# craston/object_detection_cib

Hardware: AMD Instinct MI355X
Metric: images/sec YOLOv5s 640px train (higher is better)
Workload: dtype bf16; 1 GPU; yv5s coco-zipf-like synthetic, 640px, bf16 storage/fp32 accumulate, batch 64/GPU, fwd+assign+loss+bwd+SGD, targets 4-30 boxes/img; global_batch=64, parallelism=dp1, launch=hipGraph replay, collectives=none, launcher=none, attempt=0

## Files before the change

object_detection_cib_amd/csrc/bn_act.hip:

```cpp
#include "kodhip_common.h"
#include <stdlib.h>

namespace {

__device__ __forceinline__ double wave_sum_partials(const float* p, int T, int lane) {
  double a0 = 0.0, a1 = 0.0, a2 = 0.0, a3 = 0.0;
  const int T4 = ((reinterpret_cast<uintptr_t>(p) & 15) == 0) ? (T & ~3) : 0;
#pragma unroll 4
  for (int t = lane * 4; t < T4; t += 256) {
    f32x4 v = *reinterpret_cast<const f32x4*>(p + t);
    a0 += (double)v[0]; a1 += (double)v[1]; a2 += (double)v[2]; a3 += (double)v[3];
  }
  for (int t = T4 + lane; t < T; t += 64) a0 += (double)p[t];
  return wave_sum_d((a0 + a1) + (a2 + a3));
}

__device__ __forceinline__ void wave_sum_partials2(const float* p, const float* q, int T, int lane, double& sp, double& sq) {
  const bool al = ((reinterpret_cast<uintptr_t>(p) | reinterpret_cast<uintptr_t>(q)) & 15) == 0;
  if (!al || T > 4 * 256) {
    sp = wave_sum_partials(p, T, lane);
    sq = wave_sum_partials(q, T, lane);
    return;
  }
  const int T4 = T & ~3;
// ... 59 lines not shown

__device__ __forceinline__ float bn_affine(double var, float eps, float g, float b, double mean, float* scale, float* shift) {
  float rstd = (float)(1.0 / sqrt(var + (double)eps));
  float sc = g * rstd;
  *scale = sc;
  *shift = b - (float)mean * sc;
  return rstd;
}

__device__ __forceinline__ void bn_finalize_channel(double s0, double s1, double count, float g, float b, float rm0, float rv0,
                                                    float momentum, float eps, int update_running, int c, float* scale,
                                                    float* shift, float* mean_out, float* rstd_out, float* running_mean,
                                                    float* running_var) {
  double mean = s0 / count;
  double var = s1 / count - mean * mean;
  if (var < 0.0) var = 0.0;
  float rstd = bn_affine(var, eps, g, b, mean, &scale[c], &shift[c]);
  mean_out[c] = (float)mean;
  rstd_out[c] = rstd;
  if (update_running) {
    double unbiased = count > 1.0 ? var * count / (count - 1.0) : var;
    running_mean[c] = (1.f - momentum) * rm0 + momentum * (float)mean;
    running_var[c] = (1.f - momentum) * rv0 + momentum * (float)unbiased;
  }
}

__device__ __forceinline__ double bn_central_moment(double rs, double mu, double s0, double s1) { return rs * (s1 - mu * s0); }

struct BnCoef { float k1, k2, k3; };
__device__ __forceinline__ void bn_coef_store(float* coef, int C, int c, BnCoef k) {
  coef[c] = k.k1;
  coef[C + c] = k.k2;
  coef[2 * C + c] = k.k3;
}

__device__ __forceinline__ BnCoef bn_coef_train(double g, double rs, double mu, double s0, double s1, double count) {
  double S0 = s0 / count, S1 = s1 / count;
  return {(float)(g * rs), (float)(-g * rs * rs * S1), (float)(-g * rs * S0 + g * rs * rs * mu * S1)};
}

__device__ __forceinline__ BnCoef bn_coef_eval(float g, float rstd) { return {(float)((double)g * (double)rstd), 0.f, 0.f}; }

__global__ void bn_finalize_kernel(const double* sums, double count, const float* gamma, const float* beta,
                                   float* running_mean, float* running_var, float momentum, float eps,
                                   float* scale, float* shift, float* mean_out, float* rstd_out, int C,
                                   int update_running) {
  int c = blockIdx.x * blockDim.x + threadIdx.x;
  if (c >= C) return;
  bn_finalize_channel(sums[c], sums[C + c], count, gamma[c], beta[c], update_running ? running_mean[c] : 0.f,
                      update_running ? running_var[c] : 0.f, momentum, eps, update_running, c, scale, shift, mean_out,
                      rstd_out, running_mean, running_var);
}

template <bool PEER>
__global__ void bn_finalize_fused_kernel(const float* part, int T, double count, const float* gamma,
                                         const float* beta, float* running_mean, float* running_var,
                                         float momentum, float eps, float* scale, float* shift, float* mean_out,
                                         float* rstd_out, int C, int update_running, KodPeerView pv, unsigned int slot) {
  int c = blockIdx.x * (blockDim.x >> 6) + (threadIdx.x >> 6);
  if (c >= C) return;
  int lane = threadIdx.x & 63;
  const float* p0 = part + (size_t)c * T;
  const float* p1 = part + (size_t)(C + c) * T;
  const float g = gamma[c], b = beta[c];
  const float rm0 = update_running ? running_mean[c] : 0.f, rv0 = update_running ? running_var[c] : 0.f;
  double s0, s1;
  wave_sum_partials2(p0, p1, T, lane, s0, s1);
  if constexpr (PEER) peer_allreduce2(pv, slot, c, C + c, lane, s0, s1);
  if (lane != 0) return;
  bn_finalize_channel(s0, s1, count, g, b, rm0, rv0, momentum, eps, update_running, c, scale, shift, mean_out, rstd_out,
                      running_mean, running_var);
}

struct CoefJob { const float* part; int T; double count; const float* gamma; const float* mean; const float* rstd;
                 float* dgamma; float* dbeta; float* coef; int C; int raw_moment; int eval; };

template <bool PEER>
__device__ __forceinline__ void bn_bwd_coeffs_channel(const float* part, int T, double count, const float* gamma,
                                                      const float* mean, const float* rstd, float* dgamma, float* dbeta,
                                                      float* coef, int C, int raw_moment, int eval, int c, int lane,
                                                      const KodPeerView& pv, unsigned int slot) {
  const float* p0 = part + (size_t)c * T;
  const float* p1 = part + (size_t)(C + c) * T;
  const float g_ = gamma[c], rs_ = rstd[c], mu_ = mean[c];
  double s0, s1;
  wave_sum_partials2(p0, p1, T, lane, s0, s1);
  if (raw_moment) s1 = bn_central_moment((double)rs_, (double)mu_, s0, s1);
  if (lane == 0) {
    dbeta[c] = (float)s0;
    dgamma[c] = (float)s1;
  }
  if constexpr (PEER) peer_allreduce2(pv, slot, c, C + c, lane, s0, s1);
  if (lane != 0) return;
  BnCoef k = bn_coef_train(g_, rs_, mu_, s0, s1, count);
  if (!PEER && eval) k = bn_coef_eval(g_, rs_);
  bn_coef_store(coef, C, c, k);
}

template <bool PEER>
__global__ void bn_bwd_coeffs_fused_kernel(CoefJob j0, CoefJob j1, KodPeerView pv, unsigned int slot) {
  const CoefJob& j = blockIdx.y == 0 ? j0 : j1;
  int c = blockIdx.x * (blockDim.x >> 6) + (threadIdx.x >> 6);
  if (c >= j.C) return;
  bn_bwd_coeffs_channel<PEER>(j.part, j.T, j.count, j.gamma, j.mean, j.rstd, j.dgamma, j.dbeta, j.coef, j.C, j.raw_moment,
                              j.eval, c, threadIdx.x & 63, pv, slot);
}

struct BnEvalDesc {
  const float* gamma; const float* beta; const float* running_mean; const float* running_var;
  float* aff; float* coef; long long C; long long reserved;
};

__global__ __launch_bounds__(256) void bn_eval_constants_kernel(const BnEvalDesc* desc, float eps) {
  const BnEvalDesc d = desc[blockIdx.x];
  const int C = (int)d.C;
  for (int c = threadIdx.x; c < C; c += blockDim.x) {
    const float g = d.gamma[c], b = d.beta[c], rm = d.running_mean[c];
    const float rstd = bn_affine((double)d.running_var[c], eps, g, b, (double)rm, &d.aff[c], &d.aff[C + c]);
    d.aff[2 * C + c] = rm;
    d.aff[3 * C + c] = rstd;
    if (d.coef != nullptr) bn_coef_store(d.coef, C, c, bn_coef_eval(g, rstd));
  }
}

constexpr int U = 4;

template <int ACT, int U, bool LDSK, int MAXT>
__global__ __launch_bounds__(MAXT) void bn_silu_apply_kernel(const bf16_t* y, int ldy, const float* scale, const float* shift,
                                     const bf16_t* res, int ldr, int rcoff,
                                     bf16_t* out, int ldo, int ocoff, long M, int C, int rows_per_block_iter, float slope) {
  extern __shared__ float kconst[];
  const int CC = C >> 3;
  const int cc = threadIdx.x % CC;
  const int rl = threadIdx.x / CC;
  float sc[8], sh[8];
  if (LDSK) {
    for (int c = threadIdx.x; c < C; c += blockDim.x) { kconst[c] = scale[c]; kconst[C + c] = shift[c]; }
    __syncthreads();
#pragma unroll
    for (int e = 0; e < 8; ++e) { sc[e] = kconst[cc * 8 + e]; sh[e] = kconst[C + cc * 8 + e]; }
  }
  if (rl >= rows_per_block_iter) return;
  if (!LDSK) {
#pragma unroll
    for (int e = 0; e < 8; ++e) { sc[e] = scale[cc * 8 + e]; sh[e] = shift[cc * 8 + e]; }
  }
  const long step = (long)gridDim.x * rows_per_block_iter * U;
  for (long m0 = (long)blockIdx.x * rows_per_block_iter * U + rl; m0 < M; m0 += step) {
    bf16x8 v[U], r[U];
#pragma unroll
    for (int u = 0; u < U; ++u) {
      const long m = m0 + (long)u * rows_per_block_iter;
      if (m < M) {
        v[u] = kod_load_once<bf16x8>(y + m * ldy + cc * 8);
        if (res) r[u] = *reinterpret_cast<const bf16x8*>(res + m * ldr + rcoff + cc * 8);
      }
    }
#pragma unroll
// ... 190 lines not shown
  int rpb = max_threads / CC;
  int q = 1;
  while ((q * C * 2) % 128) q *= 2;
  if (rpb >= q) rpb -= rpb % q;
  if (rpb < 1) rpb = 1;
  Geo g;
  g.rpb = rpb;
  g.threads = ((rpb * CC + 63) / 64) * 64;
  long blocks = (M + (long)rpb * U - 1) / ((long)rpb * U);
  g.grid = (int)(blocks < max_blocks ? blocks : max_blocks);
  if (g.grid < 1) g.grid = 1;
  return g;
}

#define KOD_APPLY_DISPATCH(L)                                                                              \
  do {                                                                                                     \
    const bool big = g.threads > 256;                                                                      \
    if (a.u == 4) { if (a.lds) L(4, true, 256); else L(4, false, 256); }                                   \
    else if (a.u == 2) { if (big) { if (a.lds) L(2, true, 1024); else L(2, false, 1024); }                 \
                         else { if (a.lds) L(2, true, 256); else L(2, false, 256); } }                     \
    else { if (big) { if (a.lds) L(1, true, 1024); else L(1, false, 1024); }                               \
           else { if (a.lds) L(1, true, 256); else L(1, false, 256); } }                                   \
  } while (0)

}

extern "C" {

int kodhip_bn_reduce_partials(const float* partials, double* sums, int C, int T, hipStream_t stream) {
  KOD_CHECK_ARG(partials && sums && C > 0 && T > 0, "bn_reduce_partials: bad args");
  hipLaunchKernelGGL(bn_reduce_partials_kernel, dim3(cdiv(2 * C, 4)), dim3(256), 0, stream, partials, sums, C, T);
  KOD_LAUNCH_CHECK("bn_reduce_partials");
  return KOD_OK;
}

int kodhip_bn_finalize(const double* sums, double count, const float* gamma, const float* beta,
                       float* running_mean, float* running_var, float momentum, float eps,
                       float* scale, float* shift, float* mean, float* rstd, int C, int update_running,
                       hipStream_t stream) {
  KOD_CHECK_ARG(sums && gamma && beta && scale && shift && mean && rstd && C > 0 && count > 0, "bn_finalize: bad args");
  KOD_CHECK_ARG(!update_running || (running_mean && running_var), "bn_finalize: running stats missing");
  hipLaunchKernelGGL(bn_finalize_kernel, dim3(cdiv(C, 64)), dim3(64), 0, stream, sums, count, gamma, beta,
                     running_mean, running_var, momentum, eps, scale, shift, mean, rstd, C, update_running);
  KOD_LAUNCH_CHECK("bn_finalize");
  return KOD_OK;
}

static int bn_finalize_partials(const char* fn, const float* partials, int T, double count, const float* gamma,
                                const float* beta, float* running_mean, float* running_var, float momentum, float eps,
                                float* scale, float* shift, float* mean, float* rstd, int C, int update_running,
                                const void* view, unsigned int slot, hipStream_t stream) {
  KOD_CHECK_ARG(partials && gamma && beta && scale && shift && mean && rstd && C > 0 && T > 0 && count > 0, "%s: bad args", fn);
  KOD_CHECK_ARG(!update_running || (running_mean && running_var), "%s: running stats missing", fn);
  const dim3 grid(cdiv(C, 4)), blk(256);
  if (view) {
    const KodPeerView pv = *(const KodPeerView*)view;
    KOD_CHECK_ARG(pv.world >= 1 && pv.world <= KOD_PEER_MAX && pv.world * 4 <= 64, "%s: bad peer view", fn);
    hipLaunchKernelGGL(bn_finalize_fused_kernel<true>, grid, blk, 0, stream, partials, T, count, gamma, beta, running_mean,
                       running_var, momentum, eps, scale, shift, mean, rstd, C, update_running, pv, slot);
  } else {
    hipLaunchKernelGGL(bn_finalize_fused_kernel<false>, grid, blk, 0, stream, partials, T, count, gamma, beta, running_mean,
                       running_var, momentum, eps, scale, shift, mean, rstd, C, update_running, KodPeerView{}, 0u);
  }
  KOD_LAUNCH_CHECK(fn);
  return KOD_OK;
}

static int bn_bwd_coeffs_partials(const char* fn, const CoefJob* jobs, int n_jobs, const void* view, unsigned int slot,
                                  hipStream_t stream) {
  int Cmax = 0;
  for (int i = 0; i < n_jobs; ++i) {
    const CoefJob& j = jobs[i];
    KOD_CHECK_ARG(j.part && j.gamma && j.mean && j.rstd && j.dgamma && j.dbeta && j.coef && j.C > 0 && j.T > 0 &&
                  (j.eval || j.count > 0), "%s: bad args", fn);
    if (j.C > Cmax) Cmax = j.C;
  }
  const dim3 grid(cdiv(Cmax, 4), n_jobs), blk(256);
  const CoefJob& j1 = jobs[n_jobs - 1];
  if (view) {
    const KodPeerView pv = *(const KodPeerView*)view;
    KOD_CHECK_ARG(pv.world >= 1 && pv.world <= KOD_PEER_MAX, "%s: bad peer view", fn);
    hipLaunchKernelGGL(bn_bwd_coeffs_fused_kernel<true>, grid, blk, 0, stream, jobs[0], j1, pv, slot);
  } else {
    hipLaunchKernelGGL(bn_bwd_coeffs_fused_kernel<false>, grid, blk, 0, stream, jobs[0], j1, KodPeerView{}, 0u);
  }
  KOD_LAUNCH_CHECK(fn);
  return KOD_OK;
}

int kodhip_bn_finalize_partials(const float* partials, int T, double count, const float* gamma, const float* beta,
                                float* running_mean, float* running_var, float momentum, float eps,
                                float* scale, float* shift, float* mean, float* rstd, int C, int update_running,
                                hipStream_t stream) {
  return bn_finalize_partials("bn_finalize_partials", partials, T, count, gamma, beta, running_mean, running_var, momentum, eps,
                              scale, shift, mean, rstd, C, update_running, nullptr, 0u, stream);
}

int kodhip_bn_finalize_partials_peer(const float* partials, int T, double count, const float* gamma, const float* beta,
                                     float* running_mean, float* running_var, float momentum, float eps,
                                     float* scale, float* shift, float* mean, float* rstd, int C, int update_running,
                                     const void* view, unsigned int slot, hipStream_t stream) {
  KOD_CHECK_ARG(view, "bn_finalize_partials_peer: bad args");
  return bn_finalize_partials("bn_finalize_partials_peer", partials, T, count, gamma, beta, running_mean, running_var, momentum,
                              eps, scale, shift, mean, rstd, C, update_running, view, slot, stream);
}

int kodhip_bn_bwd_coeffs_partials_peer(const float* partials, int T, double count, const float* gamma, const float* mean,
                                       const float* rstd, float* dgamma, float* dbeta, float* coef, int C,
                                       int raw_moment, const void* view, unsigned int slot, hipStream_t stream) {
  KOD_CHECK_ARG(view, "bn_bwd_coeffs_partials_peer: bad args");
  const CoefJob j = {partials, T, count, gamma, mean, rstd, dgamma, dbeta, coef, C, raw_moment, 0};
  return bn_bwd_coeffs_partials("bn_bwd_coeffs_partials_peer", &j, 1, view, slot, stream);
}

int kodhip_bn_bwd_coeffs_partials(const float* partials, int T, double count, const float* gamma, const float* mean,
                                  const float* rstd, float* dgamma, float* dbeta, float* coef, int C,
                                  int raw_moment, hipStream_t stream) {
  const CoefJob j = {partials, T, count, gamma, mean, rstd, dgamma, dbeta, coef, C, raw_moment, 0};
  return bn_bwd_coeffs_partials("bn_bwd_coeffs_partials", &j, 1, nullptr, 0u, stream);
}

int kodhip_bn_bwd_coeffs_partials2(const float* partials0, int T0, double count0, const float* gamma0, const float* mean0,
                                   const float* rstd0, float* dgamma0, float* dbeta0, float* coef0, int C0, int raw_moment0,
                                   const float* partials1, int T1, double count1, const float* gamma1, const float* mean1,
                                   const float* rstd1, float* dgamma1, float* dbeta1, float* coef1, int C1, int raw_moment1,
                                   hipStream_t stream) {
  const CoefJob j[2] = {{partials0, T0, count0, gamma0, mean0, rstd0, dgamma0, dbeta0, coef0, C0, raw_moment0, 0},
                        {partials1, T1, count1, gamma1, mean1, rstd1, dgamma1, dbeta1, coef1, C1, raw_moment1, 0}};
  return bn_bwd_coeffs_partials("bn_bwd_coeffs_partials2", j, 2, nullptr, 0u, stream);
}
// ... 144 lines not shown
```

object_detection_cib_amd/csrc/loss.hip:

```cpp
#include "kodhip_common.h"
#include "kodhip_iou.h"
#include <limits.h>

namespace {

struct AssignLevel {
  int* idx;
  int* label;
  float* gt;
  float* anc;
  int* count;
  float aw[3], ah[3];
  float fmap_w, fmap_h;
  int fw, fh;
  double inv_stride;
};
struct AssignArgs {
  AssignLevel lv[3];
  const double* boxes;
  const long* labels;
  const int* samples;
  int n, cap;
  float threshold;
};
// ... 319 lines not shown
    }
  }
  float s = block_sum_256(acc, sm);
  if (threadIdx.x == 0) a.partials[((size_t)(lvl * 3 + 1)) * a.nblk + blockIdx.x] = s;
}

__global__ void loss_scatter_kernel(LossArgs a) {
  const LossLevel& L = a.lv[blockIdx.y];
  const int m = min(*L.count, a.cap);
  int r = blockIdx.x * blockDim.x + threadIdx.x;
  if (r >= m) return;
  const int cell = cell_of(L, a.A, a.cap, r);
  if (L.last[cell] != r) return;
  const int W = 4 + a.nc;
  float* g = L.grad + (size_t)cell * a.P;
  int rows[8];
  int cnt = 0, done = -1;
  for (;;) {
    int nxt = INT_MAX;
    for (int q = L.first[cell]; q >= 0; q = L.prev[q])
      if (q > done && q < nxt) nxt = q;
    if (nxt == INT_MAX) break;
#pragma unroll
    for (int i = 0; i < 8; ++i)
      if (i == cnt) rows[i] = nxt;
    ++cnt;
    done = nxt;
  }
  if (cnt <= 8) {
    for (int k = 0; k < W; ++k) {
      float s = 0.f;
#pragma unroll
      for (int i = 0; i < 8; ++i)
        if (i < cnt) s += L.G[(size_t)rows[i] * W + k];
      g[k < 4 ? k : k + 1] = s;
    }
  } else {
    for (int k = 0; k < W; ++k) {
      float s = 0.f;
      int d2 = -1;
      for (;;) {
        int nxt = INT_MAX;
        for (int q = L.first[cell]; q >= 0; q = L.prev[q])
          if (q > d2 && q < nxt) nxt = q;
        if (nxt == INT_MAX) break;
        s += L.G[(size_t)nxt * W + k];
        d2 = nxt;
      }
      g[k < 4 ? k : k + 1] = s;
    }
  }
}

__global__ void loss_finalize_kernel(LossArgs a, int nblk_rows, int nblk_cells) {
  const int lane = threadIdx.x;
  double box = 0, obj = 0, cls = 0;
  for (int l = 0; l < 3; ++l) {
    const LossLevel& L = a.lv[l];
    double sb = 0, so = 0, sc = 0;
    for (int i = lane; i < nblk_rows; i += 64) {
      sb += (double)a.partials[(size_t)(l * 3 + 0) * a.nblk + i];
      sc += (double)a.partials[(size_t)(l * 3 + 2) * a.nblk + i];
    }
    for (int i = lane; i < nblk_cells; i += 64) so += (double)a.partials[(size_t)(l * 3 + 1) * a.nblk + i];
    sb = wave_sum_d(sb); sc = wave_sum_d(sc); so = wave_sum_d(so);
    int m = min(*L.count, a.cap);
    double ncells = (double)a.B * a.A * L.fh * L.fw;
    float lb = (float)(sb / (double)m);
    float lc = (float)(sc / ((double)m * a.nc));
    float lo = L.balance * (float)(so / ncells);
    if (lane == 0) { a.out[3 + l * 3 + 0] = lb; a.out[3 + l * 3 + 1] = lo; a.out[3 + l * 3 + 2] = lc; }
    box += lb; obj += lo; cls += lc;
  }
  if (lane == 0) {
    const float o0 = a.lam_box * (float)box, o1 = a.lam_obj * (float)obj, o2 = a.lam_cls * (float)cls;
    a.out[0] = o0;
    a.out[1] = o1;
    a.out[2] = o2;
    if (a.upstream) a.out[12] = a.upstream[0] * ((o0 + o2) + o1);
  }
}

}

extern "C" {

struct KodAssignLevel {
  int* idx; int* label; float* gt; float* anc; int* count;
  float anchor_w[3], anchor_h[3];
  int stride;
};

int kodhip_assign_targets(const double* boxes, const long* labels, const int* samples, int n, int cap,
                          int img_w, int img_h, float threshold, const KodAssignLevel* levels ,
                          hipStream_t stream) {
  KOD_CHECK_ARG(levels && cap > 0 && n >= 0, "assign_targets: bad args");
  KOD_CHECK_ARG(n == 0 || (boxes && labels && samples), "assign_targets: null inputs");
  AssignArgs a = {};
  for (int l = 0; l < 3; ++l) {
    const KodAssignLevel& s = levels[l];
    KOD_CHECK_ARG(s.idx && s.label && s.gt && s.anc && s.count && s.stride > 0, "assign_targets: bad level %d", l);
    AssignLevel& d = a.lv[l];
    d.idx = s.idx; d.label = s.label; d.gt = s.gt; d.anc = s.anc; d.count = s.count;
    for (int k = 0; k < 3; ++k) { d.aw[k] = s.anchor_w[k]; d.ah[k] = s.anchor_h[k]; }
    d.fmap_w = (float)((double)img_w / s.stride); d.fmap_h = (float)((double)img_h / s.stride);
    d.fw = img_w / s.stride; d.fh = img_h / s.stride;
    d.inv_stride = 1.0 / (double)s.stride;
  }
  a.boxes = boxes; a.labels = labels; a.samples = samples; a.n = n; a.cap = cap; a.threshold = threshold;
  hipLaunchKernelGGL(assign_kernel, dim3(3), dim3(1024), 0, stream, a);
  KOD_LAUNCH_CHECK("assign_targets");
  return KOD_OK;
}

struct KodLossLevel {
  const float* logits; float* grad;
  const int* idx; const int* label; const float* gt; const float* anc; const int* count;
  int* cellmaps;
  int* rowprev;
  float* rowgrad;
  float* tobj;
  int fh, fw;
  float balance;
};

int kodhip_yolo_loss_iou(const KodLossLevel* levels, int B, int A, int nc, int cap, float lam_box, float lam_obj, float lam_cls,
                         const float* pos_weight, const float* upstream, float* partials, int nslots, float* out,
// ... 3 lines not shown
                     float lam_box, float lam_obj, float lam_cls, const float* pos_weight,
                     const float* upstream, float* partials, int nslots, float* out, int compute_grad,
                     hipStream_t stream) {
  return kodhip_yolo_loss_iou(levels, B, A, nc, cap, lam_box, lam_obj, lam_cls, pos_weight, upstream, partials, nslots, out,
                              compute_grad, 3, 1e-7f, stream);
}

int kodhip_yolo_loss_iou(const KodLossLevel* levels , int B, int A, int nc, int cap,
                         float lam_box, float lam_obj, float lam_cls, const float* pos_weight,
                         const float* upstream, float* partials, int nslots, float* out, int compute_grad,
                         int iou_kind, float iou_eps, hipStream_t stream) {
  KOD_CHECK_ARG(levels && partials && out && B > 0 && A > 0 && nc > 0 && cap > 0, "yolo_loss: bad args");
  KOD_CHECK_ARG(iou_kind >= 0 && iou_kind <= 3 && iou_eps >= 0.f, "yolo_loss: bad IoU kind %d / eps", iou_kind);
  LossArgs a = {};
  a.iou_kind = iou_kind; a.iou_eps = iou_eps; a.iou_generic = !(iou_kind == 3 && iou_eps == 1e-7f);
  long max_cells = 0;
  for (int l = 0; l < 3; ++l) {
    const KodLossLevel& s = levels[l];
    KOD_CHECK_ARG(s.logits && s.idx && s.label && s.gt && s.anc && s.count && s.cellmaps && s.rowprev && s.rowgrad && s.tobj,
                  "yolo_loss: null pointer in level %d", l);
    KOD_CHECK_ARG(!compute_grad || s.grad, "yolo_loss: grad buffer missing");
    long ncells = (long)B * A * s.fh * s.fw;
    KOD_CHECK_ARG(ncells * (5 + nc) < (1l << 31), "yolo_loss: level too large");
    LossLevel& d = a.lv[l];
    d.logits = s.logits; d.grad = s.grad; d.idx = s.idx; d.label = s.label; d.gt = s.gt; d.anc = s.anc;
    d.count = s.count; d.last = s.cellmaps; d.first = s.cellmaps + ncells; d.cnt = s.cellmaps + 2 * ncells;
    d.G = s.rowgrad; d.tobj = s.tobj; d.prev = s.rowprev; d.fh = s.fh; d.fw = s.fw; d.balance = s.balance;
    if (ncells > max_cells) max_cells = ncells;
  }
  int nblk_rows = cdiv(cap, 256);
  int nblk_cells = 1024;
  KOD_CHECK_ARG(nslots >= nblk_rows && nslots >= nblk_cells, "yolo_loss: partials too small (%d)", nslots);
  a.B = B; a.A = A; a.nc = nc; a.P = 5 + nc; a.cap = cap;
  a.lam_box = lam_box; a.lam_obj = lam_obj; a.lam_cls = lam_cls;
  a.pos_weight = pos_weight; a.upstream = upstream; a.partials = partials; a.nblk = nslots; a.out = out;
  a.compute_grad = compute_grad;
  KOD_CHECK_ARG(5 + nc <= 128, "yolo_loss: at most 123 classes");
  a.magic_p = magic_u32((uint32_t)(5 + nc));
  for (int l = 0; l < 3; ++l) {
    long ncells = (long)B * A * a.lv[l].fh * a.lv[l].fw;
    hipError_t e1 = hipMemsetAsync(a.lv[l].last, 0xFF, 2 * ncells * sizeof(int), stream);
    if (e1 != hipSuccess) { kodhip_set_error("yolo_loss: memset failed"); return 1; }
  }
  hipLaunchKernelGGL(loss_mark_kernel, dim3(nblk_rows, 3), dim3(256), 0, stream, a);
  KOD_LAUNCH_CHECK("loss_mark");
  hipLaunchKernelGGL(loss_rows_kernel, dim3(nblk_rows, 3), dim3(256), 0, stream, a);
  KOD_LAUNCH_CHECK("loss_rows");
  hipLaunchKernelGGL(loss_cells_kernel, dim3(nblk_cells, 3), dim3(256), 0, stream, a);
  KOD_LAUNCH_CHECK("loss_cells");
  if (compute_grad) {
    hipLaunchKernelGGL(loss_scatter_kernel, dim3(nblk_rows, 3), dim3(256), 0, stream, a);
    KOD_LAUNCH_CHECK("loss_scatter");
  }
  hipLaunchKernelGGL(loss_finalize_kernel, dim3(1), dim3(64), 0, stream, a, nblk_rows, nblk_cells);
  KOD_LAUNCH_CHECK("loss_finalize");
  return KOD_OK;
}

}
```

object_detection_cib_amd/csrc/misc_ops.hip:

```cpp
#include "kodhip_common.h"

namespace {

__global__ void nchw_to_nhwc4_kernel(const float* x, bf16_t* y, int B, int C, long HW) {
  long i = (long)blockIdx.x * blockDim.x + threadIdx.x;
  if (i >= (long)B * HW) return;
  long b = i / HW, p = i - b * HW;
  bf16x4 v;
#pragma unroll
  for (int c = 0; c < 4; ++c) v[c] = (bf16_t)(c < C ? x[(b * C + c) * HW + p] : 0.f);
  *reinterpret_cast<bf16x4*>(y + i * 4) = v;
}

__global__ void nchw_to_nhwc4_x4_kernel(const float* x, bf16_t* y, int B, int C, long HW) {
  const long q = (long)blockIdx.x * blockDim.x + threadIdx.x;
  const long HWq = HW >> 2;
  if (q >= (long)B * HWq) return;
  const long b = q / HWq, pq = q - b * HWq;
  f32x4 pl[4];
#pragma unroll
  for (int c = 0; c < 4; ++c)
    pl[c] = c < C ? kod_load_once<f32x4>(x + (b * C + c) * HW + pq * 4) : f32x4{0.f, 0.f, 0.f, 0.f};
  bf16x8 o0, o1;
  const float* f0 = reinterpret_cast<const float*>(&pl[0]);
// ... 323 lines not shown

__global__ __launch_bounds__(256) void maxpool_k_bwd_kernel(const bf16_t* dy, int ldy, int ycoff, const unsigned char* idx,
                                                            bf16_t* dx, int ldx, int xcoff, int B, int H, int W, int C, int K,
                                                            const float* dx32) {
  const int C8 = C >> 3;
  const long i = (long)blockIdx.x * blockDim.x + threadIdx.x;
  if (i >= (long)B * H * W * C8) return;
  const int c8 = (int)(i % C8);
  const long p = i / C8;
  const int ix = (int)(p % W), iy = (int)((p / W) % H), b = (int)(p / ((long)W * H));
  const int r = K >> 1;
  float acc[8];
  bf16_t* d = dx + p * ldx + xcoff + c8 * 8;
  if (dx32) {
#pragma unroll
    for (int e = 0; e < 8; ++e) acc[e] = dx32[p * ldx + xcoff + c8 * 8 + e];
  } else {
    const bf16x8 old = *reinterpret_cast<const bf16x8*>(d);
#pragma unroll
    for (int e = 0; e < 8; ++e) acc[e] = (float)old[e];
  }
  for (int oy = max(iy - r, 0); oy <= min(iy + r, H - 1); ++oy)
    for (int ox = max(ix - r, 0); ox <= min(ix + r, W - 1); ++ox) {
      const long q = (long)(b * H + oy) * W + ox;
      const unsigned long long ib = *reinterpret_cast<const unsigned long long*>(idx + q * C + c8 * 8);
      const bf16x8 g = *reinterpret_cast<const bf16x8*>(dy + q * ldy + ycoff + c8 * 8);
      const unsigned me = (unsigned)((iy - oy + r) * 16 + (ix - ox + r));
#pragma unroll
      for (int e = 0; e < 8; ++e)
        if (((ib >> (8 * e)) & 0xffu) == me) acc[e] += (float)g[e];
    }
  bf16x8 o;
#pragma unroll
  for (int e = 0; e < 8; ++e) o[e] = (bf16_t)acc[e];
  *reinterpret_cast<bf16x8*>(d) = o;
}

__global__ void upsample2x_fwd_kernel(const bf16_t* x, int ldx, int xcoff, bf16_t* y, int ldy, int ycoff,
                                      int B, int H, int W, int C) {
  const int CC = C >> 3;
  long i = (long)blockIdx.x * blockDim.x + threadIdx.x;
  long total = (long)B * 4 * H * W * CC;
  if (i >= total) return;
  int cc = (int)(i % CC);
  long p = i / CC;
  int ox = (int)(p % (2 * W));
  long q = p / (2 * W);
  int oy = (int)(q % (2 * H));
  int b = (int)(q / (2 * H));
  bf16x8 v = *reinterpret_cast<const bf16x8*>(x + ((long)(b * H + (oy >> 1)) * W + (ox >> 1)) * ldx + xcoff + cc * 8);
  *reinterpret_cast<bf16x8*>(y + p * ldy + ycoff + cc * 8) = v;
}

__global__ void upsample2x_bwd_kernel(const bf16_t* dy, int ldy, int ycoff, bf16_t* dx, int ldx, int xcoff,
                                      int accumulate, int B, int H, int W, int C, const float* dx32) {
  const int CC = C >> 3;
  long i = (long)blockIdx.x * blockDim.x + threadIdx.x;
  long total = (long)B * H * W * CC;
  if (i >= total) return;
  int cc = (int)(i % CC);
  long p = i / CC;
  int ix = (int)(p % W);
  long q = p / W;
  int iy = (int)(q % H);
  int b = (int)(q / H);
  float acc[8];
  bf16_t* d = dx + p * ldx + xcoff + cc * 8;
  if (accumulate && dx32) {
    const float* o32 = dx32 + p * ldx + xcoff + cc * 8;
#pragma unroll
    for (int e = 0; e < 8; ++e) acc[e] = o32[e];
  } else if (accumulate) {
    bf16x8 old = *reinterpret_cast<const bf16x8*>(d);
#pragma unroll
    for (int e = 0; e < 8; ++e) acc[e] = (float)old[e];
  } else {
#pragma unroll
    for (int e = 0; e < 8; ++e) acc[e] = 0.f;
  }
#pragma unroll
  for (int s = 0; s < 4; ++s) {
    long op = (long)(b * 2 * H + 2 * iy + (s >> 1)) * (2 * W) + 2 * ix + (s & 1);
    bf16x8 g = *reinterpret_cast<const bf16x8*>(dy + op * ldy + ycoff + cc * 8);
#pragma unroll
    for (int e = 0; e < 8; ++e) acc[e] += (float)g[e];
  }
  bf16x8 o;
#pragma unroll
  for (int e = 0; e < 8; ++e) o[e] = (bf16_t)acc[e];
  *reinterpret_cast<bf16x8*>(d) = o;
}

__global__ __launch_bounds__(256) void head_bwd_prep_kernel(const float* g, bf16_t* dy, float* bpart, int B, int HW,
                                                            int A, int nc, int Npad, uint32_t magic_p, int PREP_ROWS) {
  extern __shared__ float sm[];
  const int P = 5 + nc;
  const int N = A * P;
  const int ldt = Npad + 1;
  const long M = (long)B * HW;
  const int ntiles = (int)((M + PREP_ROWS - 1) / PREP_ROWS);
  float bsum = 0.f;
  for (int i = threadIdx.x; i < PREP_ROWS * ldt; i += blockDim.x) sm[i] = 0.f;
  __syncthreads();
  for (int t = blockIdx.x; t < ntiles; t += gridDim.x) {
    const long m0 = (long)t * PREP_ROWS;
    const int b0 = (int)(m0 / HW), pix0 = (int)(m0 - (long)b0 * HW);
    constexpr int UNR = 4;
    const int per_an = PREP_ROWS * P;
    for (int an = 0; an < A; ++an)
      for (int base = 0; base < per_an; base += UNR * blockDim.x) {
        float v[UNR];
        int dst[UNR];
#pragma unroll
        for (int u = 0; u < UNR; ++u) {
          const int idx = base + u * blockDim.x + threadIdx.x;
          v[u] = 0.f; dst[u] = -1;
          if (idx < per_an) {
            const int r = (int)__umulhi((uint32_t)idx, magic_p);
            const int slot = idx - r * P;
            if (m0 + r < M) {
              int b = b0, pix = pix0 + r;
              while (pix >= HW) { pix -= HW; ++b; }
              v[u] = g[(((long)b * A + an) * HW + pix) * P + slot];
            }
            dst[u] = r * ldt + (slot < 4 ? 4 * an + slot : (slot == 4 ? 4 * A + an : 5 * A + an * nc + slot - 5));
          }
        }
#pragma unroll
        for (int u = 0; u < UNR; ++u)
          if (dst[u] >= 0) sm[dst[u]] = v[u];
      }
    __syncthreads();
    const int cpr = Npad / 8;
    for (int c = threadIdx.x; c < PREP_ROWS * cpr; c += blockDim.x) {
      const int r = c / cpr, n0 = (c - r * cpr) * 8;
      if (m0 + r < M) {
        bf16x8 o;
#pragma unroll
        for (int e = 0; e < 8; ++e) o[e] = (bf16_t)sm[r * ldt + n0 + e];
        *reinterpret_cast<bf16x8*>(dy + (m0 + r) * Npad + n0) = o;
      }
    }
    if (threadIdx.x < Npad) {
      float s = 0.f;
      for (int r = 0; r < PREP_ROWS; ++r) s += sm[r * ldt + threadIdx.x];
      bsum += s;
    }
    __syncthreads();
  }
  if (threadIdx.x < Npad) bpart[(size_t)blockIdx.x * Npad + threadIdx.x] = bsum;
  (void)N;
}

__global__ void head_bias_reduce_kernel(const float* bpart, int nblk, int Npad, float* db_box, float* db_obj,
                                        float* db_cls, int A, int nc) {
  int n = blockIdx.x * (blockDim.x >> 6) + (threadIdx.x >> 6);
  int lane = threadIdx.x & 63;
  int N = A * (5 + nc);
  if (n >= N) return;
  double s = 0.0;
  for (int b = lane; b < nblk; b += 64) s += (double)bpart[(size_t)b * Npad + n];
  s = wave_sum_d(s);
  if (lane != 0) return;
  if (n < 4 * A) db_box[n] = (float)s;
  else if (n < 5 * A) db_obj[n - 4 * A] = (float)s;
  else db_cls[n - 5 * A] = (float)s;
}

#define KOD_CLIP_FLOATS 16
#define KOD_NORM_BLOCKS 1024
enum { KOD_CLIP_NONE = -1, KOD_CLIP_NORM = 0, KOD_CLIP_VALUE = 1 };

template <bool NT>
__global__ __launch_bounds__(256) void grad_norm_partial_kernel(const float* __restrict__ g, const unsigned char* __restrict__ gid,
                                                                const unsigned char* __restrict__ count, long n,
                                                                const float* __restrict__ hyper, double* __restrict__ part) {
  const float gscale = hyper[9];
  double s0 = 0.0, s1 = 0.0, s2 = 0.0;
  const long stride = (long)gridDim.x * 256 * 4;
  for (long i0 = ((long)blockIdx.x * 256 + threadIdx.x) * 4; i0 < n; i0 += 4 * stride) {
    f32x4 gv[4];
    unsigned int kv[4];
    unsigned char grp[4];
#pragma unroll
    for (int u = 0; u < 4; ++u) {
      const long i = i0 + u * stride;
      const bool in = i < n;
      const long ic = in ? i : 0;
      grp[u] = gid[ic >> 6];
      kv[u] = count ? *reinterpret_cast<const unsigned int*>(count + ic) : 0x01010101u;
      gv[u] = NT ? kod_load_once<f32x4>(g + ic) : *reinterpret_cast<const f32x4*>(g + ic);
      if (!in || grp[u] > 2) kv[u] = 0;
    }
#pragma unroll
    for (int u = 0; u < 4; ++u) {
      double t = 0.0;
#pragma unroll
      for (int e = 0; e < 4; ++e) {
        const double d = (double)(gv[u][e] * gscale);
        t += ((kv[u] >> (8 * e)) & 0xffu) ? d * d : 0.0;
      }
      s0 += grp[u] == 0 ? t : 0.0;
      s1 += grp[u] == 1 ? t : 0.0;
      s2 += grp[u] == 2 ? t : 0.0;
    }
  }
  __shared__ double sm[3][4];
  s0 = wave_sum_d(s0); s1 = wave_sum_d(s1); s2 = wave_sum_d(s2);
  const int wave = threadIdx.x >> 6;
  if ((threadIdx.x & 63) == 0) { sm[0][wave] = s0; sm[1][wave] = s1; sm[2][wave] = s2; }
  __syncthreads();
  if (threadIdx.x < 3)
    part[(size_t)blockIdx.x * 3 + threadIdx.x] = (sm[threadIdx.x][0] + sm[threadIdx.x][1]) + (sm[threadIdx.x][2] + sm[threadIdx.x][3]);
}
// ... 120 lines not shown
  return KOD_OK;
}

int kodhip_maxpool5_bwd(const void* dy, int ldy, int ycoff, const void* idx, void* dx, int ldx, int xcoff,
                        int B, int H, int W, int C, const float* dx_f32, hipStream_t stream) {
  KOD_CHECK_ARG(dy && dx && idx && C % 8 == 0 && ldx % 8 == 0 && ldy % 8 == 0 && xcoff % 8 == 0 && ycoff % 8 == 0,
                "maxpool5_bwd: bad args");
  long n = (long)B * ((H + 3) / 4) * ((W + 3) / 4) * (C / 4);
  hipLaunchKernelGGL(maxpool5_bwd_kernel, dim3(cdiv(n, POOL_BWD_THREADS)), dim3(POOL_BWD_THREADS), 0, stream, (const bf16_t*)dy, ldy, ycoff,
                     (const unsigned char*)idx, (bf16_t*)dx, ldx, xcoff, B, H, W, C, dx_f32);
  KOD_LAUNCH_CHECK("maxpool5_bwd");
  return KOD_OK;
}

int kodhip_maxpool_fwd(const void* x, int ldx, int xcoff, void* y, int ldy, int ycoff, void* idx,
                       int B, int H, int W, int C, int K, hipStream_t stream) {
  if (K == 5) return kodhip_maxpool5_fwd(x, ldx, xcoff, y, ldy, ycoff, idx, B, H, W, C, stream);
  KOD_CHECK_ARG(x && y && idx && C % 8 == 0 && ldx % 8 == 0 && ldy % 8 == 0 && xcoff % 8 == 0 && ycoff % 8 == 0, "maxpool_fwd: bad args");
  KOD_CHECK_ARG(K >= 1 && K <= 15 && (K & 1), "maxpool_fwd: window %d (odd sizes up to 15)", K);
  const long n = (long)B * H * W * (C / 8);
  hipLaunchKernelGGL(maxpool_k_fwd_kernel, dim3(cdiv(n, 256)), dim3(256), 0, stream, (const bf16_t*)x, ldx, xcoff, (bf16_t*)y, ldy, ycoff,
                     (unsigned char*)idx, B, H, W, C, K);
  KOD_LAUNCH_CHECK("maxpool_fwd");
  return KOD_OK;
}

int kodhip_maxpool_bwd(const void* dy, int ldy, int ycoff, const void* idx, void* dx, int ldx, int xcoff,
                       int B, int H, int W, int C, int K, const float* dx_f32, hipStream_t stream) {
  if (K == 5) return kodhip_maxpool5_bwd(dy, ldy, ycoff, idx, dx, ldx, xcoff, B, H, W, C, dx_f32, stream);
  KOD_CHECK_ARG(dy && dx && idx && C % 8 == 0 && ldx % 8 == 0 && ldy % 8 == 0 && xcoff % 8 == 0 && ycoff % 8 == 0, "maxpool_bwd: bad args");
  KOD_CHECK_ARG(K >= 1 && K <= 15 && (K & 1), "maxpool_bwd: window %d (odd sizes up to 15)", K);
  const long n = (long)B * H * W * (C / 8);
  hipLaunchKernelGGL(maxpool_k_bwd_kernel, dim3(cdiv(n, 256)), dim3(256), 0, stream, (const bf16_t*)dy, ldy, ycoff, (const unsigned char*)idx,
                     (bf16_t*)dx, ldx, xcoff, B, H, W, C, K, dx_f32);
  KOD_LAUNCH_CHECK("maxpool_bwd");
  return KOD_OK;
}

int kodhip_upsample2x_fwd(const void* x, int ldx, int xcoff, void* y, int ldy, int ycoff,
                          int B, int H, int W, int C, hipStream_t stream) {
  KOD_CHECK_ARG(x && y && C % 8 == 0 && ldx % 8 == 0 && ldy % 8 == 0 && xcoff % 8 == 0 && ycoff % 8 == 0,
                "upsample2x_fwd: bad args");
  long n = (long)B * 4 * H * W * (C / 8);
  hipLaunchKernelGGL(upsample2x_fwd_kernel, dim3(cdiv(n, 256)), dim3(256), 0, stream, (const bf16_t*)x, ldx, xcoff,
                     (bf16_t*)y, ldy, ycoff, B, H, W, C);
  KOD_LAUNCH_CHECK("upsample2x_fwd");
  return KOD_OK;
}

int kodhip_upsample2x_bwd(const void* dy, int ldy, int ycoff, void* dx, int ldx, int xcoff, int accumulate,
                          int B, int H, int W, int C, const float* dx_f32, hipStream_t stream) {
  KOD_CHECK_ARG(dy && dx && C % 8 == 0 && ldx % 8 == 0 && ldy % 8 == 0 && xcoff % 8 == 0 && ycoff % 8 == 0,
                "upsample2x_bwd: bad args");
  long n = (long)B * H * W * (C / 8);
  hipLaunchKernelGGL(upsample2x_bwd_kernel, dim3(cdiv(n, 256)), dim3(256), 0, stream, (const bf16_t*)dy, ldy, ycoff,
                     (bf16_t*)dx, ldx, xcoff, accumulate, B, H, W, C, dx_f32);
  KOD_LAUNCH_CHECK("upsample2x_bwd");
  return KOD_OK;
}

int kodhip_head_bwd_prep(const float* g, void* dy, float* workspace, float* db_box, float* db_obj, float* db_cls,
                         int B, int HW, int A, int nc, int Npad, hipStream_t stream) {
  KOD_CHECK_ARG(g && dy && workspace && db_box && db_obj && db_cls, "head_bwd_prep: null pointer");
  KOD_CHECK_ARG(Npad % 8 == 0 && Npad >= A * (5 + nc) && Npad <= 256, "head_bwd_prep: bad Npad");
  KOD_CHECK_ARG(nc > 0 && 5 + nc <= 128, "head_bwd_prep: bad class count");
  long M = (long)B * HW;
  const int PREP_ROWS = Npad <= 128 ? 64 : 32;
  int grid = (int)((M + PREP_ROWS - 1) / PREP_ROWS);
  if (grid > 2048) grid = 2048;
  hipLaunchKernelGGL(head_bwd_prep_kernel, dim3(grid), dim3(256), PREP_ROWS * (Npad + 1) * sizeof(float), stream, g,
                     (bf16_t*)dy, workspace, B, HW, A, nc, Npad, magic_u32((uint32_t)(5 + nc)), PREP_ROWS);
  KOD_LAUNCH_CHECK("head_bwd_prep");
  hipLaunchKernelGGL(head_bias_reduce_kernel, dim3(cdiv(A * (5 + nc), 4)), dim3(256), 0, stream,
                     (const float*)workspace, grid, Npad, db_box, db_obj, db_cls, A, nc);
  KOD_LAUNCH_CHECK("head_bias_reduce");
  return KOD_OK;
}

static int sgd_nesterov(const char* fn, float* params, const float* grads, float* momentum_buf, const void* group_ids,
                        const void* keep_mask, long n, const float* hyper, const float* clip, int mode, int skip_nonfinite,
                        hipStream_t stream) {
  KOD_CHECK_ARG(params && grads && momentum_buf && group_ids && hyper && n > 0 && n % 64 == 0, "%s: bad args", fn);
  KOD_CHECK_ARG(!clip || mode == KOD_CLIP_NORM || mode == KOD_CLIP_VALUE, "%s: unknown mode %d", fn, mode);
  const int cl = clip ? mode : KOD_CLIP_NONE;
#define KOD_SGD(M, CL) \
  hipLaunchKernelGGL((sgd_nesterov_kernel<M, CL>), dim3(cdiv(n / 4, 256)), dim3(256), 0, stream, params, grads, momentum_buf, \
                     (const unsigned char*)group_ids, (const unsigned char*)keep_mask, n, hyper, clip, skip_nonfinite)
#define KOD_SGD_CLIP(M)                                                                                              \
  do {                                                                                                               \
    if (cl == KOD_CLIP_NONE) KOD_SGD(M, KOD_CLIP_NONE); else if (cl == KOD_CLIP_NORM) KOD_SGD(M, KOD_CLIP_NORM); else KOD_SGD(M, KOD_CLIP_VALUE); \
  } while (0)
  if (keep_mask) KOD_SGD_CLIP(true); else KOD_SGD_CLIP(false);
#undef KOD_SGD_CLIP
#undef KOD_SGD
  KOD_LAUNCH_CHECK(fn);
  return KOD_OK;
}

int kodhip_sgd_nesterov(float* params, const float* grads, float* momentum_buf, const void* group_ids,
                        long n, const float* hyper, hipStream_t stream) {
  return sgd_nesterov("sgd_nesterov", params, grads, momentum_buf, group_ids, nullptr, n, hyper, nullptr, 0, 0, stream);
}

int kodhip_sgd_nesterov_masked(float* params, const float* grads, float* momentum_buf, const void* group_ids,
                               const void* keep_mask, long n, const float* hyper, hipStream_t stream) {
  KOD_CHECK_ARG(keep_mask, "sgd_nesterov_masked: bad args");
  return sgd_nesterov("sgd_nesterov_masked", params, grads, momentum_buf, group_ids, keep_mask, n, hyper, nullptr, 0, 0, stream);
}

// ... 76 lines not shown
```

Before: 5579 images/sec.

## Tune small reduction kernels, parallelize loss finalize, restructure upsample backward indexing

Several unrelated small-kernel changes land together. The BN stat kernels now clamp out-of-range channels instead of exiting early, and hoist scalar arguments with an empty asm. loss_finalize runs one wave per level instead of looping over levels, using unrolled strided loads. head_bias_reduce gets a 16-way unrolled load loop. upsample2x_bwd switches to a 2D grid indexed by row, which avoids 64-bit div/mod, and issues all four gradient loads up front. The aim is lower latency in these short, latency-bound kernels, paid for with extra register pressure and more complex code.

Result: no change. 5576 images/sec, median of 2 (-0.1%).

```diff
diff --git a/object_detection_cib_amd/csrc/bn_act.hip b/object_detection_cib_amd/csrc/bn_act.hip
--- a/object_detection_cib_amd/csrc/bn_act.hip
+++ b/object_detection_cib_amd/csrc/bn_act.hip
@@ -135,22 +135,33 @@
                       rstd_out, running_mean, running_var);
 }
 
+constexpr int STAT_WAVES = 4;
+#define KOD_ARGS_NOW(...) asm volatile("" ::__VA_ARGS__)
+
 template <bool PEER>
-__global__ void bn_finalize_fused_kernel(const float* part, int T, double count, const float* gamma,
+__global__ __launch_bounds__(64 * STAT_WAVES) void bn_finalize_fused_kernel(const float* part, int T, double count, const float* gamma,
                                          const float* beta, float* running_mean, float* running_var,
                                          float momentum, float eps, float* scale, float* shift, float* mean_out,
                                          float* rstd_out, int C, int update_running, KodPeerView pv, unsigned int slot) {
-  int c = blockIdx.x * (blockDim.x >> 6) + (threadIdx.x >> 6);
-  if (c >= C) return;
+  int c = blockIdx.x * STAT_WAVES + (threadIdx.x >> 6);
+  const bool live = c < C;
+  if constexpr (PEER) { if (!live) return; }
+  else {
+    c = live ? c : C - 1;
+    KOD_ARGS_NOW("s"(count), "s"(momentum), "s"(eps), "s"(scale), "s"(shift), "s"(mean_out), "s"(rstd_out));
+  }
   int lane = threadIdx.x & 63;
   const float* p0 = part + (size_t)c * T;
   const float* p1 = part + (size_t)(C + c) * T;
+  const float* rmp = update_running ? running_mean : gamma;
+  const float* rvp = update_running ? running_var : gamma;
   const float g = gamma[c], b = beta[c];
-  const float rm0 = update_running ? running_mean[c] : 0.f, rv0 = update_running ? running_var[c] : 0.f;
+  float rm0 = rmp[c], rv0 = rvp[c];
   double s0, s1;
   wave_sum_partials2(p0, p1, T, lane, s0, s1);
+  if (!update_running) rm0 = rv0 = 0.f;
   if constexpr (PEER) peer_allreduce2(pv, slot, c, C + c, lane, s0, s1);
-  if (lane != 0) return;
+  if (lane != 0 || !live) return;
   bn_finalize_channel(s0, s1, count, g, b, rm0, rv0, momentum, eps, update_running, c, scale, shift, mean_out, rstd_out,
                       running_mean, running_var);
 }
@@ -162,31 +173,34 @@
 __device__ __forceinline__ void bn_bwd_coeffs_channel(const float* part, int T, double count, const float* gamma,
                                                       const float* mean, const float* rstd, float* dgamma, float* dbeta,
                                                       float* coef, int C, int raw_moment, int eval, int c, int lane,
-                                                      const KodPeerView& pv, unsigned int slot) {
+                                                      bool live, const KodPeerView& pv, unsigned int slot) {
+  if constexpr (!PEER) KOD_ARGS_NOW("s"(count), "s"(dgamma), "s"(dbeta), "s"(coef), "s"(raw_moment), "s"(eval));
   const float* p0 = part + (size_t)c * T;
   const float* p1 = part + (size_t)(C + c) * T;
   const float g_ = gamma[c], rs_ = rstd[c], mu_ = mean[c];
   double s0, s1;
   wave_sum_partials2(p0, p1, T, lane, s0, s1);
   if (raw_moment) s1 = bn_central_moment((double)rs_, (double)mu_, s0, s1);
-  if (lane == 0) {
+  if (lane == 0 && live) {
     dbeta[c] = (float)s0;
     dgamma[c] = (float)s1;
   }
   if constexpr (PEER) peer_allreduce2(pv, slot, c, C + c, lane, s0, s1);
-  if (lane != 0) return;
+  if (lane != 0 || !live) return;
   BnCoef k = bn_coef_train(g_, rs_, mu_, s0, s1, count);
   if (!PEER && eval) k = bn_coef_eval(g_, rs_);
   bn_coef_store(coef, C, c, k);
 }
 
 template <bool PEER>
-__global__ void bn_bwd_coeffs_fused_kernel(CoefJob j0, CoefJob j1, KodPeerView pv, unsigned int slot) {
+__global__ __launch_bounds__(64 * STAT_WAVES) void bn_bwd_coeffs_fused_kernel(CoefJob j0, CoefJob j1, KodPeerView pv, unsigned int slot) {
   const CoefJob& j = blockIdx.y == 0 ? j0 : j1;
-  int c = blockIdx.x * (blockDim.x >> 6) + (threadIdx.x >> 6);
-  if (c >= j.C) return;
+  int c = blockIdx.x * STAT_WAVES + (threadIdx.x >> 6);
+  const bool live = c < j.C;
+  if constexpr (PEER) { if (!live) return; }
+  else c = live ? c : j.C - 1;
   bn_bwd_coeffs_channel<PEER>(j.part, j.T, j.count, j.gamma, j.mean, j.rstd, j.dgamma, j.dbeta, j.coef, j.C, j.raw_moment,
-                              j.eval, c, threadIdx.x & 63, pv, slot);
+                              j.eval, c, threadIdx.x & 63, live, pv, slot);
 }
 
 struct BnEvalDesc {
@@ -483,7 +497,7 @@
                                 const void* view, unsigned int slot, hipStream_t stream) {
   KOD_CHECK_ARG(partials && gamma && beta && scale && shift && mean && rstd && C > 0 && T > 0 && count > 0, "%s: bad args", fn);
   KOD_CHECK_ARG(!update_running || (running_mean && running_var), "%s: running stats missing", fn);
-  const dim3 grid(cdiv(C, 4)), blk(256);
+  const dim3 grid(cdiv(C, STAT_WAVES)), blk(64 * STAT_WAVES);
   if (view) {
     const KodPeerView pv = *(const KodPeerView*)view;
     KOD_CHECK_ARG(pv.world >= 1 && pv.world <= KOD_PEER_MAX && pv.world * 4 <= 64, "%s: bad peer view", fn);
@@ -506,7 +520,7 @@
                   (j.eval || j.count > 0), "%s: bad args", fn);
     if (j.C > Cmax) Cmax = j.C;
   }
-  const dim3 grid(cdiv(Cmax, 4), n_jobs), blk(256);
+  const dim3 grid(cdiv(Cmax, STAT_WAVES), n_jobs), blk(64 * STAT_WAVES);
   const CoefJob& j1 = jobs[n_jobs - 1];
   if (view) {
     const KodPeerView pv = *(const KodPeerView*)view;
diff --git a/object_detection_cib_amd/csrc/loss.hip b/object_detection_cib_amd/csrc/loss.hip
--- a/object_detection_cib_amd/csrc/loss.hip
+++ b/object_detection_cib_amd/csrc/loss.hip
@@ -395,27 +395,53 @@
   }
 }
 
-__global__ void loss_finalize_kernel(LossArgs a, int nblk_rows, int nblk_cells) {
-  const int lane = threadIdx.x;
-  double box = 0, obj = 0, cls = 0;
-  for (int l = 0; l < 3; ++l) {
+constexpr int FIN_U = 16;
+__device__ __forceinline__ void lane_sums_strided(const float* pb, const float* pc, const float* po, int nr, int no, int lane,
+                                                  double& sb, double& sc, double& so) {
+  sb = sc = so = 0;
+  const int nmax = max(nr, no);
+  for (int i0 = lane; i0 < nmax; i0 += 64 * FIN_U) {
+    float vb[FIN_U], vc[FIN_U], vo[FIN_U];
+#pragma unroll
+    for (int u = 0; u < FIN_U; ++u) {
+      const int ir = min(i0 + 64 * u, nr - 1), io = min(i0 + 64 * u, no - 1);
+      vb[u] = pb[ir]; vc[u] = pc[ir]; vo[u] = po[io];
+    }
+#pragma unroll
+    for (int u = 0; u < FIN_U; ++u) {
+      const double tb = sb + (double)vb[u], tc = sc + (double)vc[u], to = so + (double)vo[u];
+      sb = i0 + 64 * u < nr ? tb : sb;
+      sc = i0 + 64 * u < nr ? tc : sc;
+      so = i0 + 64 * u < no ? to : so;
+    }
+  }
+}
+
+__global__ __launch_bounds__(192) void loss_finalize_kernel(LossArgs a, int nblk_rows, int nblk_cells) {
+  __shared__ float lvl_mean[3][3];
+  const int lane = threadIdx.x & 63;
+  const int l = __builtin_amdgcn_readfirstlane(threadIdx.x >> 6);
+  {
     const LossLevel& L = a.lv[l];
-    double sb = 0, so = 0, sc = 0;
-    for (int i = lane; i < nblk_rows; i += 64) {
-      sb += (double)a.partials[(size_t)(l * 3 + 0) * a.nblk + i];
-      sc += (double)a.partials[(size_t)(l * 3 + 2) * a.nblk + i];
-    }
-    for (int i = lane; i < nblk_cells; i += 64) so += (double)a.partials[(size_t)(l * 3 + 1) * a.nblk + i];
+    const int cnt = *L.count;
+    const float* pl = a.partials + (size_t)(l * 3) * a.nblk;
+    double sb, sc, so;
+    lane_sums_strided(pl, pl + 2 * (size_t)a.nblk, pl + (size_t)a.nblk, nblk_rows, nblk_cells, lane, sb, sc, so);
     sb = wave_sum_d(sb); sc = wave_sum_d(sc); so = wave_sum_d(so);
-    int m = min(*L.count, a.cap);
+    int m = min(cnt, a.cap);
     double ncells = (double)a.B * a.A * L.fh * L.fw;
     float lb = (float)(sb / (double)m);
     float lc = (float)(sc / ((double)m * a.nc));
     float lo = L.balance * (float)(so / ncells);
-    if (lane == 0) { a.out[3 + l * 3 + 0] = lb; a.out[3 + l * 3 + 1] = lo; a.out[3 + l * 3 + 2] = lc; }
-    box += lb; obj += lo; cls += lc;
-  }
-  if (lane == 0) {
+    if (lane == 0) {
+      a.out[3 + l * 3 + 0] = lb; a.out[3 + l * 3 + 1] = lo; a.out[3 + l * 3 + 2] = lc;
+      lvl_mean[l][0] = lb; lvl_mean[l][1] = lo; lvl_mean[l][2] = lc;
+    }
+  }
+  __syncthreads();
+  if (threadIdx.x == 0) {
+    double box = 0, obj = 0, cls = 0;
+    for (int q = 0; q < 3; ++q) { box += lvl_mean[q][0]; obj += lvl_mean[q][1]; cls += lvl_mean[q][2]; }
     const float o0 = a.lam_box * (float)box, o1 = a.lam_obj * (float)obj, o2 = a.lam_cls * (float)cls;
     a.out[0] = o0;
     a.out[1] = o1;
@@ -525,7 +551,7 @@
     hipLaunchKernelGGL(loss_scatter_kernel, dim3(nblk_rows, 3), dim3(256), 0, stream, a);
     KOD_LAUNCH_CHECK("loss_scatter");
   }
-  hipLaunchKernelGGL(loss_finalize_kernel, dim3(1), dim3(64), 0, stream, a, nblk_rows, nblk_cells);
+  hipLaunchKernelGGL(loss_finalize_kernel, dim3(1), dim3(192), 0, stream, a, nblk_rows, nblk_cells);
   KOD_LAUNCH_CHECK("loss_finalize");
   return KOD_OK;
 }
diff --git a/object_detection_cib_amd/csrc/misc_ops.hip b/object_detection_cib_amd/csrc/misc_ops.hip
--- a/object_detection_cib_amd/csrc/misc_ops.hip
+++ b/object_detection_cib_amd/csrc/misc_ops.hip
@@ -399,24 +399,28 @@
   *reinterpret_cast<bf16x8*>(y + p * ldy + ycoff + cc * 8) = v;
 }
 
-__global__ void upsample2x_bwd_kernel(const bf16_t* dy, int ldy, int ycoff, bf16_t* dx, int ldx, int xcoff,
-                                      int accumulate, int B, int H, int W, int C, const float* dx32) {
-  const int CC = C >> 3;
-  long i = (long)blockIdx.x * blockDim.x + threadIdx.x;
-  long total = (long)B * H * W * CC;
-  if (i >= total) return;
-  int cc = (int)(i % CC);
-  long p = i / CC;
-  int ix = (int)(p % W);
-  long q = p / W;
-  int iy = (int)(q % H);
-  int b = (int)(q / H);
+__global__ __launch_bounds__(512) void upsample2x_bwd_kernel(const bf16_t* dy, int ldy, int ycoff, bf16_t* dx, int ldx, int xcoff,
+                                      int accumulate, int W, int CC, const float* dx32) {
+  const unsigned j = blockIdx.y * blockDim.x + threadIdx.x;
+  if (j >= (unsigned)(W * CC)) return;
+  const int ix = (int)(j / (unsigned)CC);
+  const int cc = (int)(j - (unsigned)ix * (unsigned)CC);
+  const long row = blockIdx.x;
+  const long p = row * W + ix;
+  bf16x8 g[4];
+#pragma unroll
+  for (int s = 0; s < 4; ++s) {
+    const long op = (2 * row + (s >> 1)) * (2 * W) + 2 * ix + (s & 1);
+    g[s] = kod_load_once<bf16x8>(dy + op * ldy + ycoff + cc * 8);
+  }
   float acc[8];
   bf16_t* d = dx + p * ldx + xcoff + cc * 8;
   if (accumulate && dx32) {
     const float* o32 = dx32 + p * ldx + xcoff + cc * 8;
-#pragma unroll
-    for (int e = 0; e < 8; ++e) acc[e] = o32[e];
+    typedef float f32x4u __attribute__((ext_vector_type(4), aligned(4)));
+    const f32x4u a0 = *reinterpret_cast<const f32x4u*>(o32), a1 = *reinterpret_cast<const f32x4u*>(o32 + 4);
+#pragma unroll
+    for (int e = 0; e < 4; ++e) { acc[e] = a0[e]; acc[4 + e] = a1[e]; }
   } else if (accumulate) {
     bf16x8 old = *reinterpret_cast<const bf16x8*>(d);
 #pragma unroll
@@ -427,10 +431,8 @@
   }
 #pragma unroll
   for (int s = 0; s < 4; ++s) {
-    long op = (long)(b * 2 * H + 2 * iy + (s >> 1)) * (2 * W) + 2 * ix + (s & 1);
-    bf16x8 g = *reinterpret_cast<const bf16x8*>(dy + op * ldy + ycoff + cc * 8);
-#pragma unroll
-    for (int e = 0; e < 8; ++e) acc[e] += (float)g[e];
+#pragma unroll
+    for (int e = 0; e < 8; ++e) acc[e] += (float)g[s][e];
   }
   bf16x8 o;
 #pragma unroll
@@ -505,8 +507,18 @@
   int lane = threadIdx.x & 63;
   int N = A * (5 + nc);
   if (n >= N) return;
+  constexpr int UNR = 16;
   double s = 0.0;
-  for (int b = lane; b < nblk; b += 64) s += (double)bpart[(size_t)b * Npad + n];
+  for (int b0 = lane; b0 < nblk; b0 += 64 * UNR) {
+    float v[UNR];
+#pragma unroll
+    for (int u = 0; u < UNR; ++u) v[u] = bpart[(size_t)min(b0 + 64 * u, nblk - 1) * Npad + n];
+#pragma unroll
+    for (int u = 0; u < UNR; ++u) {
+      const double t = s + (double)v[u];
+      s = b0 + 64 * u < nblk ? t : s;
+    }
+  }
   s = wave_sum_d(s);
   if (lane != 0) return;
   if (n < 4 * A) db_box[n] = (float)s;
@@ -733,9 +745,14 @@
                           int B, int H, int W, int C, const float* dx_f32, hipStream_t stream) {
   KOD_CHECK_ARG(dy && dx && C % 8 == 0 && ldx % 8 == 0 && ldy % 8 == 0 && xcoff % 8 == 0 && ycoff % 8 == 0,
                 "upsample2x_bwd: bad args");
-  long n = (long)B * H * W * (C / 8);
-  hipLaunchKernelGGL(upsample2x_bwd_kernel, dim3(cdiv(n, 256)), dim3(256), 0, stream, (const bf16_t*)dy, ldy, ycoff,
-                     (bf16_t*)dx, ldx, xcoff, accumulate, B, H, W, C, dx_f32);
+  KOD_CHECK_ARG(B > 0 && H > 0 && W > 0 && C > 0 && (long)B * H < (1l << 31) && (long)W * (C / 8) < (1l << 31),
+                "upsample2x_bwd: bad shape");
+  const long per_row = (long)W * (C / 8);
+  const int chunks = cdiv(per_row, 512);
+  const int threads = cdiv(cdiv(per_row, chunks), 64) * 64;
+  KOD_CHECK_ARG(chunks <= 65535, "upsample2x_bwd: row too wide");
+  hipLaunchKernelGGL(upsample2x_bwd_kernel, dim3((unsigned)((long)B * H), chunks), dim3(threads), 0, stream, (const bf16_t*)dy, ldy,
+                     ycoff, (bf16_t*)dx, ldx, xcoff, accumulate, W, C / 8, dx_f32);
   KOD_LAUNCH_CHECK("upsample2x_bwd");
   return KOD_OK;
 }
```
